# codename0og/codename-rvc-fork-3

Measured on AMD Instinct MI355X. Metric: 48 kHz audio samples/sec end-to-end VC, higher is better.
Workload: dtype f32 (vocoder ResBlock convs and upsamplers, HuBERT, RMVPE's U-Net convs: fp32 operands as exact bf16x3 splits on the bf16 matrix cores -- six products of order <= 2^-16 per multiply-add, fp32 accumulate; everything else fp32 / fp64)

## Files before the change

### codename-rvc-fork-3_amd/csrc/common.h

```cpp
#pragma once

#include <hip/hip_runtime.h>
#include <stdint.h>
#include <stdio.h>
#include <stdlib.h>
#include <string.h>

#include <string>

#include "bf16x3.h"
#include "rvc_amd.h"

namespace rvc {

void set_error(const char *fmt, ...);
int fail(const char *fmt, ...);

#define RVC_HIP(expr)                                                                         \
    do {                                                                                      \
        hipError_t _e = (expr);                                                               \
        if (_e != hipSuccess) return ::rvc::fail("%s failed: %s (%s:%d)", #expr, hipGetErrorString(_e), \
                                                 __FILE__, __LINE__);                         \
    } while (0)

// ... 20 lines not shown

static inline int64_t ceil_div(int64_t a, int64_t b) { return (a + b - 1) / b; }
static inline size_t align_up(size_t v, size_t a) { return (v + a - 1) / a * a; }

int cu_count();

struct PersistentGrid {
    int per_xcd;
    unsigned blocks;
};
static inline PersistentGrid persistent_grid(int64_t n_tiles) {
    const int per_xcd = (int)ceil_div(n_tiles, 8), cus_per_xcd = cu_count() / 8;
    return {per_xcd, 8u * (unsigned)(cus_per_xcd < per_xcd ? cus_per_xcd : per_xcd)};
}

static inline bool fits_2gib(int64_t elems, int elem_bytes) { return elems * elem_bytes < ((int64_t)1 << 31); }

int upload_packed(const char *fn, const void *host, size_t bytes, void *dev, void *stream);

typedef float f32x16 __attribute__((ext_vector_type(16)));
typedef float f32x4 __attribute__((ext_vector_type(4)));

__device__ __forceinline__ f32x16 mfma32(float a, float b, f32x16 c) {
    return __builtin_amdgcn_mfma_f32_32x32x2f32(a, b, c, 0, 0, 0);
}
__device__ __forceinline__ int mfma32_row(int reg, int lane) { return (reg & 3) + 8 * (reg >> 2) + 4 * (lane >> 5); }

__device__ __forceinline__ void lds_barrier() { asm volatile("s_waitcnt lgkmcnt(0)\n\ts_barrier" ::: "memory"); }

__device__ __forceinline__ float lrelu(float v, float slope) { return v > 0.f ? v : v * slope; }
// ... 3 lines not shown
```

### codename-rvc-fork-3_amd/csrc/convbf1.hip

```cpp
#include <stdlib.h>

#include <algorithm>
#include <mutex>
#include <type_traits>
#include <vector>

#include "conv.h"
#include "f16x2.h"

namespace rvc {

constexpr int CB1_NTH = 512;
constexpr int CB1_CK = 64;
constexpr int CB1_N1 = 64;

struct Cb1Bf16Taps {
    static constexpr const char *NAME = "convbf1";
    using frag = bf16x8;
    static constexpr bool PAIRS = false;
    static constexpr int PLANES = 3;
    static constexpr int TAPF = 1;
    static constexpr int NACC = 1;
    static constexpr int OUT_OPS = 24, VM_MAX = 56;
    static constexpr int tap_plane(int) { return 0; }
// ... 11 lines not shown
    static constexpr int tap_plane(int i) { return i == 2; }
    static constexpr int win_plane(int i) { return i == 0; }
    static constexpr int acc_of(int i) { return i != 1; }
};

struct Cb1Params {
    const float *x = nullptr;
    const void *u = nullptr;
    const float *bias = nullptr;
    const float *res = nullptr;
    const float *accin = nullptr;
    float *y = nullptr;
    int64_t L = 0;
    int dil = 1;
    float slope = 1.f, out_scale = 1.f;
    int tiles_per_row = 0, n_tiles = 0, per_xcd = 0;
};

template <int KW, int C, class F>
struct Cb1Geom {
    static constexpr int NCH = C / CB1_CK;
    static constexpr int RBW = C / 128;
    static constexpr int KS = CB1_CK / 16;
    static constexpr int NGC = KW * KS;
    static constexpr int NGT = NCH * NGC;
    static constexpr int H = (KW - 1) / 2;
    static constexpr int ROWB = 2 * F::PLANES * CB1_CK + 16;
    static constexpr int XROWS = CB1_N1 + (KW - 1) * 5;
    static constexpr int X_BYTES = (XROWS + 1) * ROWB;
    static constexpr int RC32 = (XROWS + 31) / 32;
    static constexpr int NIT = (CB1_CK / 8) * RC32 / 4;
    static constexpr int IO_BYTES = C * CB1_N1 * 4;
    static constexpr int LDS_BYTES = 2 * X_BYTES + IO_BYTES;
    static constexpr int ROWBLOCKS = C / 32;
    static constexpr int CONV_BYTES = NGT * ROWBLOCKS * F::TAPF * 1024;
    static constexpr int PA = F::TAPF == 1 ? 8 : 8 / RBW;
    static_assert(C == 128 || C == 256, "square layers of 128 or 256 channels");
    static_assert((CB1_CK / 8) * RC32 % 4 == 0, "the items must divide over the four stager waves");
    static_assert(4 * NIT + F::OUT_OPS <= F::VM_MAX, "memory operations in flight per stager wave");
    static_assert(LDS_BYTES <= 163840, "LDS budget");
    static_assert((ROWB / 16) % 2 == 1, "row stride must be an odd multiple of 16 bytes");
};

template <int KW, int C, class F>
__global__ void __launch_bounds__(CB1_NTH) __attribute__((amdgpu_waves_per_eu(2, 2)))
convbf1_kernel(const Cb1Params p) {
    using GM = Cb1Geom<KW, C, F>;
    using frag = typename F::frag;
    constexpr int NCH = GM::NCH, RBW = GM::RBW, KS = GM::KS, NGC = GM::NGC, NGT = GM::NGT, H = GM::H, ROWB = GM::ROWB, NIT = GM::NIT;
    constexpr int N1 = CB1_N1, CK = CB1_CK, PA = GM::PA, PLANES = F::PLANES, TAPF = F::TAPF, NACC = F::NACC;

    extern __shared__ __attribute__((aligned(16))) unsigned char cb_smem[];
    unsigned char *const xs = cb_smem;
    float *const io_lds = reinterpret_cast<float *>(cb_smem + 2 * GM::X_BYTES);

    const int tid = threadIdx.x, lane = tid & 63;
    const int wave = __builtin_amdgcn_readfirstlane(tid >> 6);
    const int half = lane >> 5, l31 = lane & 31;
    const int d = p.dil, XR = N1 + (KW - 1) * d;
    const int64_t L = p.L;
    const unsigned L4 = (unsigned)(L * 4);
    const int num_bytes = (int)((int64_t)C * L * 4);

    const int xcd = blockIdx.x & 7, slot = blockIdx.x >> 3, nslot = gridDim.x >> 3;
    const int tile_end = (xcd + 1) * p.per_xcd < p.n_tiles ? (xcd + 1) * p.per_xcd : p.n_tiles;
    const int tile0 = xcd * p.per_xcd + slot;
    if (tile0 >= tile_end) return;
    const int my_tiles = (tile_end - tile0 + nslot - 1) / nslot;
    const int n_q = my_tiles * NCH;

    if (wave >= 4) {
        __builtin_amdgcn_s_setprio(1);
        const int sw = wave - 4;
        float xr[NIT][4];
        constexpr int RC = GM::RC32;
        const int lq = lane >> 5;
        auto x_issue = [&](int q) __attribute__((always_inline)) {
            const int tl = tile0 + (q / NCH) * nslot, ch0 = (q % NCH) * CK;
            const int bb = tl / p.tiles_per_row;
            const int xt0 = (tl - bb * p.tiles_per_row) * N1 - H * d;
            const __amdgpu_buffer_rsrc_t rs = __builtin_amdgcn_make_buffer_rsrc((void *)(p.x + (int64_t)bb * C * L), 0, num_bytes, RSRC_RAW32);
            const unsigned Lu = (unsigned)L;
            int sw_o = sw;
            asm volatile("" : "+s"(sw_o));
#pragma unroll
            for (int i = 0; i < NIT; ++i) {
                const int wi = sw_o * NIT + i, qp = wi / RC, rc = wi - qp * RC;
                const int qd = 2 * qp + lq, r = rc * 32 + l31;
                const unsigned tg = (unsigned)(xt0 + r);
                const bool ok = r < XR && tg < Lu;
                const unsigned base = (unsigned)(ch0 + 4 * qd) * L4 + tg * 4u;
#pragma unroll
                for (int e = 0; e < 4; ++e)
// ... 78 lines not shown
                    }
                    if (l4) {
                        __builtin_amdgcn_raw_buffer_store_b128(__builtin_bit_cast(u32x4, f32x4{re[0], re[1], re[2], re[3]}), yrs, (int)o, 0, 0);
                    } else {
#pragma unroll
                        for (int e = 0; e < 4; ++e) {
                            const unsigned oe = (ok && t0 + 4 * chunk + e < L) ? o + 4u * (unsigned)e : BUF_OOB;
                            __builtin_amdgcn_raw_buffer_store_b32(__builtin_bit_cast(unsigned, re[e]), yrs, (int)oe, 0, 0);
                        }
                    }
                }
            }
        };
        x_issue(0);
        x_write(0);
        if (1 < n_q) x_issue(1);
        for (int q = 0; q < n_q; ++q) {
            lds_barrier();
            if (q % NCH == 0 && q > 0) out_store(tile0 + (q / NCH - 1) * nslot);
            if (q + 1 < n_q) x_write(q + 1);
            asm volatile("s_waitcnt vmcnt(8)" ::: "memory");
            if (q + 2 < n_q) x_issue(q + 2);
        }
        lds_barrier();
        out_store(tile0 + (my_tiles - 1) * nslot);
        return;
    }

    float bias[RBW][16];
    if constexpr (!F::PAIRS) {
#pragma unroll
        for (int rb = 0; rb < RBW; ++rb)
#pragma unroll
            for (int r = 0; r < 16; ++r) {
                const int ch = 32 * (RBW * wave + rb) + (r & 3) + 8 * (r >> 2) + 4 * half;
                bias[rb][r] = p.bias ? p.bias[ch] : 0.f;
            }
    }
    const __amdgpu_buffer_rsrc_t urs = __builtin_amdgcn_make_buffer_rsrc((void *)p.u, 0, GM::CONV_BYTES, RSRC_RAW32);
    frag fa[PA][RBW][TAPF];
// ... 9 lines not shown
        const int soff = (g * GM::ROWBLOCKS + RBW * wave) * TAPF * 1024;
        fa[slot_a][f / TAPF][f % TAPF] = __builtin_bit_cast(frag, __builtin_amdgcn_raw_buffer_load_b128(urs, 16 * lane + f * 1024, soff, 0));
    };
    auto load_b1 = [&](int buf, const unsigned char *src, int gc, int cb, int s) __attribute__((always_inline)) {
        const int tap = gc / KS, ks = gc - tap * KS;
        fb[buf][cb][s] = __builtin_bit_cast(frag, *reinterpret_cast<const u32x4 *>(src + tap * d * ROWB + ks * 32 + cb * 32 * ROWB + s * 2 * CK));
    };
#pragma unroll
    for (int g = 0; g < PA - 1; ++g) load_a(g, g);
    const int x_lane = l31 * ROWB + half * 16;
    float *const io_mine = io_lds + (32 * RBW * wave + 4 * half) * N1 + l31;
    constexpr int NM = 6 * RBW;

    static_assert((2 * NGC) % PA == 0 && NCH % 2 == 0, "two chunks of groups must be whole turns of the tap ring");
    int q = 0;
    for (int t = 0; t < my_tiles; ++t) {
#pragma unroll
        for (int rb = 0; rb < RBW; ++rb)
#pragma unroll
            for (int cb = 0; cb < 2; ++cb)
#pragma unroll
                for (int a = 0; a < NACC; ++a)
#pragma unroll
                    for (int r = 0; r < 16; ++r) acc[rb][cb][a][r] = 0.f;
#pragma unroll 1
        for (int cp = 0; cp < NCH / 2; ++cp) {
            const int g0 = cp * 2 * NGC;
#pragma unroll
            for (int c2 = 0; c2 < 2; ++c2, ++q) {
                lds_barrier();
                const unsigned char *const src = xs + (q & 1) * GM::X_BYTES + x_lane;
// ... 79 lines not shown
                            const int co = 32 * rb + (lane & 31), ci = CB1_CK * ch + 16 * ks + 8 * (lane >> 5) + e;
                            const size_t group = ((size_t)ch * k + tap) * KS + ks, at = (group * RB + rb) * planes * 512 + lane * 8 + e;
                            const float v = w[((size_t)co * c + ci) * k + tap];
                            if (fmt == CB1_F16X2) f16x2_split_host(v, &(*out)[at], &(*out)[at + 512]);
                            else (*out)[at] = bf16_rne(v);
                        }
    return 0;
}

template <int KW, int C, class F>
static int cb1_launch(Cb1Params p, int batch, hipStream_t stream) {
    if (reserve_whole_cu((const void *)convbf1_kernel<KW, C, F>, F::NAME)) return 1;
    p.tiles_per_row = (int)ceil_div(p.L, CB1_N1);
    p.n_tiles = p.tiles_per_row * batch;
    const PersistentGrid g = persistent_grid(p.n_tiles);
    p.per_xcd = g.per_xcd;
    hipLaunchKernelGGL((convbf1_kernel<KW, C, F>), dim3(g.blocks), dim3(CB1_NTH), LDS_WHOLE_CU, stream, p);
    RVC_LAUNCH_CHECK();
    return 0;
}

template <class F>
static int cb1_dispatch(const Cb1Params &p, int batch, int c, int k, hipStream_t stream) {
#define RVC_CB1_CASE(KW, CC) if (k == KW && c == CC) return cb1_launch<KW, CC, F>(p, batch, stream)
    RVC_CB1_CASE(3, 128); RVC_CB1_CASE(7, 128); RVC_CB1_CASE(11, 128);
    RVC_CB1_CASE(3, 256); RVC_CB1_CASE(7, 256); RVC_CB1_CASE(11, 256);
#undef RVC_CB1_CASE
    return fail("%s: unsupported shape c=%d k=%d", F::NAME, c, k);
}

int launch_convbf1(Cb1Format fmt, const float *x, const void *u, const float *bias, const float *res, const float *accin, float *y, int batch,
// ... 68 lines not shown
```

### codename-rvc-fork-3_amd/csrc/error.cpp

```cpp
#include <stdarg.h>

#include <map>
#include <mutex>
#include <unordered_map>

#include "common.h"

namespace rvc {

static thread_local char g_err[1024] = "";

void set_error(const char *fmt, ...) {
    va_list ap;
    va_start(ap, fmt);
    vsnprintf(g_err, sizeof(g_err), fmt, ap);
    va_end(ap);
}

int fail(const char *fmt, ...) {
    va_list ap;
    va_start(ap, fmt);
    vsnprintf(g_err, sizeof(g_err), fmt, ap);
    va_end(ap);
    return 1;
}

namespace {
struct DeviceState {
    int cus = 0;
    std::unordered_map<const void *, int> lds;
};
std::mutex g_dev_mu;
std::map<int, DeviceState> g_dev;
}

int reserve_lds(const void *kernel, int bytes, const char *what) {
    int dev = 0;
    RVC_HIP(hipGetDevice(&dev));
    std::lock_guard<std::mutex> g(g_dev_mu);
    int &granted = g_dev[dev].lds[kernel];
    if (bytes <= granted) return 0;
    const hipError_t e = hipFuncSetAttribute(kernel, hipFuncAttributeMaxDynamicSharedMemorySize, bytes);
    if (e != hipSuccess) return fail("%s: cannot reserve %d bytes of LDS on device %d: %s", what, bytes, dev, hipGetErrorString(e));
    granted = bytes;
    return 0;
}

int cu_count() {
    int dev = 0, cus = 0;
    if (hipGetDevice(&dev) != hipSuccess) return 256;
    std::lock_guard<std::mutex> g(g_dev_mu);
    DeviceState &d = g_dev[dev];
    if (!d.cus) d.cus = hipDeviceGetAttribute(&cus, hipDeviceAttributeMultiprocessorCount, dev) == hipSuccess && cus > 0 ? cus : 256;
    return d.cus;
}

int upload_packed(const char *fn, const void *host, size_t bytes, void *dev, void *stream) {
    hipError_t e = hipMemcpyAsync(dev, host, bytes, hipMemcpyHostToDevice, (hipStream_t)stream);
    if (e == hipSuccess) e = hipStreamSynchronize((hipStream_t)stream);
    if (e != hipSuccess) return fail("%s: %s", fn, hipGetErrorString(e));
    return 0;
}

}

extern "C" int rvc_abi_version(void) { return RVC_AMD_ABI_VERSION; }
extern "C" const char *rvc_last_error(void) { return rvc::g_err; }
```

### codename-rvc-fork-3_amd/csrc/resblock_bf.hip

```cpp
#include <stdlib.h>

#include <algorithm>
#include <atomic>
#include <mutex>
#include <type_traits>
#include <vector>

#include "conv.h"

namespace rvc {

constexpr int RBF_NTH = 512;

struct RbfParams {
    const float *x = nullptr;
    const void *u = nullptr;
    const float *b1 = nullptr, *b2 = nullptr;
    const float *accin = nullptr;
    float *y = nullptr;
    int64_t L = 0;
    int dil = 1;
    float slope = 1.f, out_scale = 1.f;
    int tiles_per_row = 0, n_tiles = 0, per_xcd = 0;
};

template <int KW, int C, int NTS = 3>
struct RbfGeom {
    static constexpr int KS = C / 16, RB = C / 32, CG = 4 / RB;
    static constexpr int N1 = CG * 64;
    static constexpr int H2 = (KW - 1) / 2;
    static constexpr int BN = (N1 - (KW - 1)) / 4 * 4;
    static constexpr int ROWB = 6 * C + 16;
    static constexpr int XROWS = N1 + (KW - 1) * 5;
    static constexpr int TROWS = N1 + (KW - 1);
    static constexpr int X_BYTES = (XROWS + 1) * ROWB, T_BYTES = TROWS * ROWB;
    static constexpr int RC32 = (XROWS + 31) / 32;
    static constexpr int NIT = (C / 8) * RC32 / 4;
    static constexpr int NG = KW * KS;
    static constexpr int GROUP_BYTES = NTS * 1024;
    static_assert(NTS == 1 || NTS == 3, "tap split: one term (bf16-valued taps) or three (fp32 taps)");
    static constexpr int CONV_BYTES = NG * RB * GROUP_BYTES;
    static constexpr int R_BYTES = C * N1 * 4 + 16;
    static constexpr int LDS_BYTES = X_BYTES + T_BYTES + R_BYTES;
    static_assert((C / 8) * RC32 % 4 == 0, "the items must divide over the four stager waves");
    static_assert(4 * NIT + 8 <= 56, "memory operations in flight per stager wave (kept below the 6-bit counter's range: see the stager's prologue)");
    static_assert(LDS_BYTES <= 163840, "LDS budget");
    static_assert((ROWB / 16) % 2 == 1, "row stride must be an odd multiple of 16 bytes");
};

template <int KW, int C, int DBG = 0, int NTS = 3>
__global__ void __launch_bounds__(RBF_NTH) __attribute__((amdgpu_waves_per_eu(2, 2)))
resblock_bf_kernel(const RbfParams p) {
    using GM = RbfGeom<KW, C, NTS>;
    constexpr int KS = GM::KS, RB = GM::RB, N1 = GM::N1, H2 = GM::H2, BN = GM::BN, ROWB = GM::ROWB, NIT = GM::NIT;
    constexpr int NG = GM::NG, PA = NTS == 1 ? 8 : 4;

    extern __shared__ __attribute__((aligned(16))) unsigned char rb_smem[];
    unsigned char *const xs = rb_smem;
    unsigned char *const ts = rb_smem + GM::X_BYTES;
    float *const io_lds = reinterpret_cast<float *>(rb_smem + GM::X_BYTES + GM::T_BYTES);

    const int tid = threadIdx.x, lane = tid & 63;
    const int wave = __builtin_amdgcn_readfirstlane(tid >> 6);
    const int half = lane >> 5, l31 = lane & 31;
    const int d = p.dil, h1 = H2 * d, XR = N1 + 2 * h1;
    const int64_t L = p.L;
    const unsigned L4 = (unsigned)(L * 4);
    const int num_bytes = (int)((int64_t)C * L * 4);

    const int xcd = blockIdx.x & 7, slot = blockIdx.x >> 3, nslot = gridDim.x >> 3;
    const int tile_end = (xcd + 1) * p.per_xcd < p.n_tiles ? (xcd + 1) * p.per_xcd : p.n_tiles;
    int tile = xcd * p.per_xcd + slot;
    if (tile >= tile_end) return;
    unsigned long long *const stamps = (DBG & 128) ? reinterpret_cast<unsigned long long *>(const_cast<float *>(p.accin)) + ((size_t)blockIdx.x * 2 + (wave >= 4 ? 1 : 0)) * 64 : nullptr;
    int n_stamp = 0;
    auto stamp = [&]() __attribute__((always_inline)) {
        if constexpr (DBG & 128) {
            if ((wave == 0 || wave == 4) && lane == 0 && n_stamp < 64) stamps[n_stamp] = __builtin_readcyclecounter();
            ++n_stamp;
        }
    };

    if (wave >= 4) {
        __builtin_amdgcn_s_setprio(1);
        const int ht = tid - 256, sw = wave - 4;
        constexpr int NSET = C == 32 ? 2 : 1;
        float xr[NSET][NIT][4];
        constexpr int RC = GM::RC32;
        const int lq = lane >> 5;
        auto x_issue = [&](auto SET, int tl) __attribute__((always_inline)) {
            constexpr int st = decltype(SET)::value;
            const int bb = tl / p.tiles_per_row;
            const int xt0 = (tl - bb * p.tiles_per_row) * BN - H2 - h1;
            const __amdgpu_buffer_rsrc_t rs = __builtin_amdgcn_make_buffer_rsrc((void *)(p.x + (int64_t)bb * C * L), 0, num_bytes, RSRC_RAW32);
            const unsigned Lu = (unsigned)L;
            int sw_o = sw;
            asm volatile("" : "+s"(sw_o));
#pragma unroll
            for (int i = 0; i < NIT; ++i) {
                const int wi = sw_o * NIT + i, qp = wi / RC, rc = wi - qp * RC;
                const int q = 2 * qp + lq, r = rc * 32 + l31;
// ... 78 lines not shown
                        re[e] = mul_np(re[e], out_scale);
                    }
                    if (l4) {
                        __builtin_amdgcn_raw_buffer_store_b128(__builtin_bit_cast(u32x4, f32x4{re[0], re[1], re[2], re[3]}), yrs, (int)o, 0, 0);
                    } else {
#pragma unroll
                        for (int e = 0; e < 4; ++e) {
                            const unsigned oe = (ok && t0 + 4 * chunk + e < L) ? o + 4u * (unsigned)e : BUF_OOB;
                            __builtin_amdgcn_raw_buffer_store_b32(__builtin_bit_cast(unsigned, re[e]), yrs, (int)oe, 0, 0);
                        }
                    }
                }
            }
        };
        const bool has_acc = p.accin != nullptr && !(DBG & 128);
        for (int o = ht * 16; o < (KW - 1) * ROWB; o += 256 * 16) *reinterpret_cast<u32x4 *>(ts + N1 * ROWB + o) = u32x4{0u, 0u, 0u, 0u};
        constexpr std::integral_constant<int, 0> S0{};
        constexpr std::integral_constant<int, NSET - 1> SL{};
        x_issue(S0, tile);
        x_write(S0);
        if (NSET == 2 && tile + nslot < tile_end) x_issue(SL, tile + nslot);
        int prev = -1;
        auto phase = [&](int tl, auto SET_CUR, auto SET_NEXT) __attribute__((always_inline)) {
            stamp();
            lds_barrier();
            stamp();
            lds_barrier();
            if (prev >= 0) out_store(prev, has_acc);
            asm volatile("s_waitcnt vmcnt(8)" ::: "memory");
            if (tl + NSET * nslot < tile_end) x_issue(SET_CUR, tl + NSET * nslot);
            stamp();
            lds_barrier();
            stamp();
            if constexpr (DBG & 128) asm volatile("s_waitcnt vmcnt(0)" ::: "memory");
            stamp();
            if (tl + nslot < tile_end) x_write(SET_NEXT);
            stamp();
            n_stamp += 2;
            prev = tl;
        };
        for (; tile < tile_end; tile += 2 * nslot) {
            phase(tile, S0, SL);
            if (tile + nslot < tile_end) phase(tile + nslot, SL, S0);
        }
        lds_barrier();
        asm volatile("s_waitcnt vmcnt(0)" ::: "memory");
        lds_barrier();
        out_store(prev, has_acc);
        return;
    }

    const int rb = wave % RB, cg = wave / RB;
    const int col0 = cg * 64;
    float bias1[16], bias2[16];
#pragma unroll
    for (int r = 0; r < 16; ++r) {
        const int ch = 32 * rb + (r & 3) + 8 * (r >> 2) + 4 * half;
        bias1[r] = p.b1 ? p.b1[ch] : 0.f;
        bias2[r] = p.b2 ? p.b2[ch] : 0.f;
    }
    const __amdgpu_buffer_rsrc_t urs = __builtin_amdgcn_make_buffer_rsrc((void *)p.u, 0, 2 * GM::CONV_BYTES, RSRC_RAW32);
    const float slope = p.slope;

// ... 58 lines not shown
#pragma unroll
        for (int cb = 0; cb < 2; ++cb)
#pragma unroll
            for (int r = 0; r < 16; ++r) rsd[cb][r] = io_mine[((r & 3) + 8 * (r >> 2)) * N1 + cb * 32];
#pragma unroll
        for (int cb = 0; cb < 2; ++cb)
#pragma unroll
            for (int r = 0; r < 16; ++r) io_mine[((r & 3) + 8 * (r >> 2)) * N1 + cb * 32] = io[cb][r];
#pragma unroll
        for (int cb = 0; cb < 2; ++cb)
#pragma unroll
            for (int r = 0; r < 16; ++r) io[cb][r] = rsd[cb][r];
    };

    a_prologue(0);
    for (; tile < tile_end; tile += nslot) {
        const int bb = tile / p.tiles_per_row;
        const int64_t t0 = (int64_t)(tile - bb * p.tiles_per_row) * BN;
        stamp();
        lds_barrier();
        stamp();
        swap_io();
        stamp();
        lds_barrier();
        stamp();
        conv_loop(0, xsrc, xstep);
        stamp();
        a_prologue(1);
#pragma unroll
        for (int cb = 0; cb < 2; ++cb) {
            const int j = col0 + cb * 32 + l31;
// ... 75 lines not shown
                            const size_t group = (((size_t)cv * k + tap) * KS + ks) * RB + rb;
                            uint16_t h[3];
                            bf16_split_host(w[((size_t)co * c + ci) * k + tap], tap_splits, h);
                            for (int s = 0; s < tap_splits; ++s) (*out)[(group * tap_splits + s) * 512 + lane * 8 + e] = h[s];
                        }
    }
}

template <int KW, int C, int DBG = 0, int NTS = 3>
static int rbf_launch(RbfParams p, int batch, hipStream_t stream) {
    using GM = RbfGeom<KW, C, NTS>;
    if (reserve_whole_cu((const void *)resblock_bf_kernel<KW, C, DBG, NTS>, "resblock_bf")) return 1;
    p.tiles_per_row = (int)ceil_div(p.L, GM::BN);
    p.n_tiles = p.tiles_per_row * batch;
    const PersistentGrid g = persistent_grid(p.n_tiles);
    p.per_xcd = g.per_xcd;
    hipLaunchKernelGGL((resblock_bf_kernel<KW, C, DBG, NTS>), dim3(g.blocks), dim3(RBF_NTH), LDS_WHOLE_CU, stream, p);
    RVC_LAUNCH_CHECK();
    return 0;
}

int launch_resblock_bf(const float *x, const void *u, const float *b1, const float *b2, const float *accin, float *y, int batch, int c,
                       int64_t L, int k, int dil, float slope, float out_scale, hipStream_t stream, int tap_splits) {
    if (!resblock_bf_supported(c, k, dil)) return fail("resblock_bf: unsupported shape (%d channels, %d taps, dilation %d)", c, k, dil);
    if (tap_splits != 1 && tap_splits != 3) return fail("resblock_bf: tap split of %d terms (1 or 3)", tap_splits);
    if (x == y) return fail("resblock_bf: in-place operation is not supported");
    if (!(slope >= 0.f && slope <= 1.f)) return fail("resblock_bf: leaky slope %g outside [0, 1]", (double)slope);
    if (!resblock_bf_fits(c, L)) return fail("resblock_bf: a %d x %lld slab exceeds the 2 GiB buffer addressing", c, (long long)L);
    if (L <= 0 || batch <= 0) return 0;
    if ((int64_t)ceil_div(L, 64) * batch >= ((int64_t)1 << 30)) return fail("resblock_bf: too many tiles");
    RbfParams p;
// ... 71 lines not shown
```

### codename-rvc-fork-3_amd/csrc/upsbf.hip

```cpp
#include <stdlib.h>

#include <algorithm>
#include <mutex>
#include <type_traits>
#include <vector>

#include "conv.h"

namespace rvc {

constexpr int UB_NTH = 512;
constexpr int UB_CK = 64;

struct UbParams {
    const float *x = nullptr;
    const float *har = nullptr;
    const void *u = nullptr;
    const float *bias = nullptr;
    float *y = nullptr;
    int64_t L_in = 0, L_out = 0, Lh = 0;
    int c_in = 0, c_out = 0;
    int n_xchunks = 0;
    int vk = 0;
    int S = 0, P = 0;
    int pad = 0;
    float slope = 0.1f;
    int n_mblk = 0, col_tiles = 0, n_tiles = 0, per_xcd = 0;
};

template <int R, int MB>
struct UbGeom {
    static constexpr int RB_T = MB / 32;
    static constexpr int RBW = RB_T >= 4 ? RB_T / 4 : 1;
    static constexpr int CG = RB_T >= 4 ? 1 : 4 / RB_T;
    static constexpr int N1 = 64 * CG;
    static constexpr int W = N1 * R;
    static constexpr int CPB = (MB - 1) / R + 2;
    static constexpr int KS = UB_CK / 16;
    static constexpr int NGC = 2 * KS;
    static constexpr int PA = 4;
    static constexpr int ROWB = 6 * UB_CK + 16;
    static constexpr int XROWS = N1 + 1;
    static constexpr int X_BYTES = (XROWS + 1) * ROWB;
    static constexpr int RC32 = (XROWS + 31) / 32;
    static constexpr int NIT = (UB_CK / 8) * RC32 / 4;
    static constexpr int IO_FLOATS = CPB * W;
    static constexpr int IO_BYTES = IO_FLOATS * 4 + 16;
    static constexpr int LDS_BYTES = 2 * X_BYTES + IO_BYTES;
    static constexpr int GROUP_BYTES = RB_T * 3 * 1024;
    static_assert(MB == 64 || MB == 128 || MB == 256, "GEMM rows per tile");
    static_assert(R >= 1 && R <= MB, "a channel's phases span at most two m-blocks");
    static_assert((UB_CK / 8) * RC32 % 4 == 0, "the items must divide over the four stager waves");
    static_assert(NGC % PA == 0 && KS % PA == 0, "a chunk's groups must be whole turns of the tap ring");
    static_assert(LDS_BYTES <= 163840, "LDS budget");
};

template <int R, int MB>
__global__ void __launch_bounds__(UB_NTH) __attribute__((amdgpu_waves_per_eu(2, 2)))
upsbf_kernel(const UbParams p) {
    using GM = UbGeom<R, MB>;
    constexpr int RB_T = GM::RB_T, RBW = GM::RBW, N1 = GM::N1, W = GM::W, KS = GM::KS, NGC = GM::NGC, PA = GM::PA, ROWB = GM::ROWB;
    constexpr int NIT = GM::NIT, CK = UB_CK;

    extern __shared__ __attribute__((aligned(16))) unsigned char ub_smem[];
    unsigned char *const xs = ub_smem;
    float *const io_lds = reinterpret_cast<float *>(ub_smem + 2 * GM::X_BYTES);

    const int tid = threadIdx.x, lane = tid & 63;
    const int wave = __builtin_amdgcn_readfirstlane(tid >> 6);
    const int half = lane >> 5, l31 = lane & 31;
    const int64_t L_in = p.L_in, L_out = p.L_out;
    const int nxc = p.n_xchunks, ncht = nxc + (p.vk > 0 ? 1 : 0);
    const int ngt = nxc * NGC + (p.vk > 0 ? KS : 0);
    const int n_mblk = p.n_mblk;
    const int m_total = p.c_out * R;

    const int xcd = blockIdx.x & 7, slot = blockIdx.x >> 3, nslot = gridDim.x >> 3;
    const int tile_end = (xcd + 1) * p.per_xcd < p.n_tiles ? (xcd + 1) * p.per_xcd : p.n_tiles;
    const int tile0 = xcd * p.per_xcd + slot;
    if (tile0 >= tile_end) return;
    const int my_tiles = (tile_end - tile0 + nslot - 1) / nslot;
    const int n_q = my_tiles * ncht;
    auto tile_coords = [&](int tl, int &mblk, int &ct, int &bb) __attribute__((always_inline)) {
        mblk = tl % n_mblk;
        const int rest = tl / n_mblk;
        bb = rest / p.col_tiles;
        ct = rest - bb * p.col_tiles;
    };

    for (int o = tid * 16; o < 2 * GM::X_BYTES; o += UB_NTH * 16) *reinterpret_cast<u32x4 *>(xs + o) = u32x4{0u, 0u, 0u, 0u};
    lds_barrier();
    const int nqp_noise = (p.vk + 1 + 7) / 8;

    if (wave >= 4) {
        __builtin_amdgcn_s_setprio(1);
        const int sw = wave - 4, ht = tid - 256;
        float xr[NIT][4];
        constexpr int RC = GM::RC32;
        const int lq = lane >> 5;
        const unsigned L4 = (unsigned)(L_in * 4);
        const int x_bytes = (int)((int64_t)p.c_in * L_in * 4);
        auto x_issue = [&](int tl, int ci) __attribute__((always_inline)) {
            int mblk, ct, bb;
            tile_coords(tl, mblk, ct, bb);
            const int q0m1 = ct * N1 - 1;
            int sw_o = sw;
// ... 77 lines not shown
                    const int64_t t = t_base + i;
                    const int m = (co0 + row) * R + i % R;
                    const bool ok = f < n_el && m >= m0 && m < m0 + MB && m < m_total && t >= 0 && t < L_out;
                    v[k] = io_lds[f < n_el ? f : 0];
                    bv[k] = !fold && p.bias && ok ? p.bias[co0 + row] : 0.f;
                    off[k] = ok ? (unsigned)(co0 + row) * Lo4 + (unsigned)t * 4u : BUF_OOB;
                }
#pragma unroll
                for (int k = 0; k < 4; ++k) __builtin_amdgcn_raw_buffer_store_b32(__builtin_bit_cast(unsigned, v[k] + bv[k]), yrs, (int)off[k], 0, 0);
            }
        };
        int wt = 0, wc = 0, it = 0, ic = 0;
        auto adv = [&](int &t_, int &c_) __attribute__((always_inline)) {
            if (++c_ == ncht) { c_ = 0; ++t_; }
        };
        x_issue(tile0, 0);
        x_write(0, 0);
        adv(wt, wc); adv(it, ic);
        if (1 < n_q) x_issue(tile0 + it * nslot, ic);
        adv(it, ic);
        int ct_i = 0, cc_i = 0;
        for (int q = 0; q < n_q; ++q) {
            lds_barrier();
            if (cc_i == 0 && q > 0) out_store(tile0 + (ct_i - 1) * nslot);
            if (ncht == 1) lds_barrier();
            if (q + 1 < n_q) x_write(q + 1, wc);
            adv(wt, wc);
            asm volatile("s_waitcnt vmcnt(8)" ::: "memory");
            if (q + 2 < n_q) x_issue(tile0 + it * nslot, ic);
            adv(it, ic);
            adv(ct_i, cc_i);
        }
        lds_barrier();
        out_store(tile0 + (my_tiles - 1) * nslot);
        return;
    }

    const int rb0 = RB_T >= 4 ? RBW * wave : wave % RB_T;
    const int col0 = RB_T >= 4 ? 0 : 64 * (wave / RB_T);
    const __amdgpu_buffer_rsrc_t urs = __builtin_amdgcn_make_buffer_rsrc((void *)p.u, 0, n_mblk * ngt * GM::GROUP_BYTES, RSRC_RAW32);
    bf16x8 fa[PA][RBW][3];
    bf16x8 fb[2][2][3];
    f32x16 acc[RBW][2];
    auto load_a1 = [&](int slot_a, int byte_off, int rb, int s) __attribute__((always_inline)) {
        fa[slot_a][rb][s] = __builtin_bit_cast(bf16x8, __builtin_amdgcn_raw_buffer_load_b128(urs, 16 * lane + ((rb0 + rb) * 3 + s) * 1024, byte_off, 0));
    };
    auto load_b1 = [&](int buf, const unsigned char *src, int gc, int cb, int s) __attribute__((always_inline)) {
        const int j = gc / KS, ks = gc - j * KS;
        fb[buf][cb][s] = __builtin_bit_cast(bf16x8, *reinterpret_cast<const u32x4 *>(src + (1 - j) * ROWB + ks * 32 + cb * 32 * ROWB + s * 2 * CK));
    };
    const int x_lane = (col0 + l31) * ROWB + half * 16;
    constexpr int ia6[6] = {0, 1, 0, 2, 1, 0}, ib6[6] = {2, 1, 1, 0, 0, 0};
    constexpr int NM = 12 * RBW;

    int mblk, ct, bb;
    tile_coords(tile0, mblk, ct, bb);
    int a_base = mblk * ngt * GM::GROUP_BYTES;
#pragma unroll
    for (int g = 0; g < PA - 1; ++g)
#pragma unroll
        for (int rb = 0; rb < RBW; ++rb)
#pragma unroll
            for (int s = 0; s < 3; ++s) load_a1(g, a_base + g * GM::GROUP_BYTES, rb, s);

    int q = 0;
    for (int t = 0; t < my_tiles; ++t) {
        const int tl = tile0 + t * nslot;
        tile_coords(tl, mblk, ct, bb);
        a_base = mblk * ngt * GM::GROUP_BYTES;
        int a_next = a_base;
        if (t + 1 < my_tiles) {
            int m2, c2, b2;
            tile_coords(tl + nslot, m2, c2, b2);
            a_next = m2 * ngt * GM::GROUP_BYTES;
        }
#pragma unroll
        for (int rb = 0; rb < RBW; ++rb)
#pragma unroll
            for (int cb = 0; cb < 2; ++cb)
#pragma unroll
                for (int r = 0; r < 16; ++r) acc[rb][cb][r] = 0.f;
        int g0 = 0;
#pragma unroll 1
        for (int c = 0; c < ncht; ++c, ++q) {
            const bool noise = c == nxc;
            lds_barrier();
            const unsigned char *const src = xs + (q & 1) * GM::X_BYTES + x_lane;
#pragma unroll
// ... 99 lines not shown
                            const int k = kq - ph * nc_stride;
                            float v = row_ok && kq < vk && k >= 0 && k < nc_k ? nw[(size_t)co * nc_k + k] : 0.f;
                            if (row_ok && kq == vk && bias) v = bias[co];
                            put((size_t)mblk * ngt + nxc * 8 + ks, rb, lane, e, v);
                        }
            }
}

template <int R, int MB>
static int ub_launch(UbParams p, int batch, hipStream_t stream) {
    using GM = UbGeom<R, MB>;
    if (reserve_whole_cu((const void *)upsbf_kernel<R, MB>, "upsbf")) return 1;
    p.col_tiles = (int)ceil_div(p.L_in + 1, GM::N1);
    p.n_tiles = p.col_tiles * p.n_mblk * batch;
    const PersistentGrid g = persistent_grid(p.n_tiles);
    p.per_xcd = g.per_xcd;
    hipLaunchKernelGGL((upsbf_kernel<R, MB>), dim3(g.blocks), dim3(UB_NTH), LDS_WHOLE_CU, stream, p);
    RVC_LAUNCH_CHECK();
    return 0;
}

int launch_upsbf(const float *x, const float *har, int64_t Lh, const void *u, const float *bias, float *y, int batch, int c_in, int c_out,
                 int64_t L_in, int64_t L_out, int rate, int ksize, int pad, int vk, int64_t S, int64_t P, float slope, hipStream_t stream) {
    if (!upsbf_supported(c_in, c_out, rate, ksize, vk)) return fail("upsbf: unsupported shape (%d -> %d channels, rate %d, kernel %d, %d noise rows)", c_in, c_out, rate, ksize, vk);
    if (vk > 0 && (!har || Lh <= 0 || !fits_2gib(Lh, 4) || S > 4096 || P > 65536)) return fail("upsbf: bad noise source");
    if (!fits_2gib((int64_t)c_in * L_in, 4) || !fits_2gib((int64_t)c_out * L_out, 4)) return fail("upsbf: slab exceeds the 2 GiB buffer addressing");
    if (L_in <= 0 || batch <= 0) return 0;
    UbParams p;
    p.x = x; p.har = har; p.u = u; p.bias = bias; p.y = y; p.L_in = L_in; p.L_out = L_out; p.Lh = vk > 0 ? Lh : 0;
    p.c_in = c_in; p.c_out = c_out; p.n_xchunks = c_in / UB_CK; p.vk = vk; p.S = (int)S; p.P = (int)P; p.pad = pad; p.slope = slope;
    int mb, ngt;
// ... 50 lines not shown
```

Measured before the change: 61.46 million.

## Replace static persistent tile striding with atomic per-XCD tile claiming and work stealing

Persistent conv, resblock and upsampler kernels now take tiles dynamically from per-XCD atomic counters instead of a fixed stride. Each block prefers its home XCD's range and steals from other XCDs once that range runs dry. Tile indices go into a small LDS ring so the stager and MFMA waves can prefetch ahead, and the last block to finish resets the counters. The aim is to cut tail imbalance between blocks, at the cost of atomic traffic, extra readfirstlane LDS reads and a per-stream counter pool.

```diff
diff --git a/codename-rvc-fork-3_amd/csrc/common.h b/codename-rvc-fork-3_amd/csrc/common.h
--- a/codename-rvc-fork-3_amd/csrc/common.h
+++ b/codename-rvc-fork-3_amd/csrc/common.h
@@ -58,6 +58,107 @@
     return {per_xcd, 8u * (unsigned)(cus_per_xcd < per_xcd ? cus_per_xcd : per_xcd)};
 }
 
+constexpr int CLAIM_WORDS = 16, CLAIM_DONE = 8;
+struct TileClaim {
+    unsigned *ctr = nullptr;
+    int n_tiles = 0, per_xcd = 0;
+};
+int tile_claim_counters(hipStream_t stream, unsigned **ctr);
+static inline int tile_claim(hipStream_t stream, int64_t n_tiles, const PersistentGrid &g, TileClaim *c) {
+    c->n_tiles = (int)n_tiles;
+    c->per_xcd = g.per_xcd;
+    c->ctr = nullptr;
+    if (!knob("RVC_TILE_CLAIM", 1)) return 0;
+    return tile_claim_counters(stream, &c->ctr);
+}
+
+#ifdef __HIPCC__
+struct TileClaimer {
+    int home = 0, tried = 0;
+    unsigned left = 0xffu;
+    int next = 0, step = 0, end = 0;
+};
+__device__ __forceinline__ TileClaimer tile_claimer(const TileClaim &c) {
+    TileClaimer s;
+    s.home = blockIdx.x & 7;
+    const int hi = (s.home + 1) * c.per_xcd;
+    s.next = s.home * c.per_xcd + (int)(blockIdx.x >> 3);
+    s.step = (int)(gridDim.x >> 3);
+    s.end = hi < c.n_tiles ? hi : c.n_tiles;
+    return s;
+}
+__device__ __forceinline__ void claim_range(const TileClaim &c, const TileClaimer &s, int &x, int &lo, int &len) {
+    x = (s.home + s.tried) & 7;
+    lo = x * c.per_xcd;
+    const int hi = lo + c.per_xcd < c.n_tiles ? lo + c.per_xcd : c.n_tiles;
+    len = hi > lo ? hi - lo : 0;
+}
+__device__ __forceinline__ unsigned claim_issue(const TileClaim &c, TileClaimer &s) {
+#ifdef RVC_ABLATE
+    if (!c.ctr) return 0u;
+#endif
+    while (s.tried < 8) {
+        int x, lo, len;
+        claim_range(c, s, x, lo, len);
+        if (len > 0 && (s.left >> x & 1u)) return atomicAdd(c.ctr + x, 1u);
+        ++s.tried;
+    }
+    return 0u;
+}
+__device__ __forceinline__ int claim_take(const TileClaim &c, TileClaimer &s, unsigned drawn) {
+#ifdef RVC_ABLATE
+    if (!c.ctr) {
+        const int t = s.next;
+        s.next += s.step;
+        return t < s.end ? t : -1;
+    }
+#endif
+    while (s.tried < 8) {
+        int x, lo, len;
+        claim_range(c, s, x, lo, len);
+        if (drawn < (unsigned)len) return lo + (int)drawn;
+        if (s.tried++ == 0) {
+            unsigned seen[8];
+#pragma unroll
+            for (int r = 0; r < 8; ++r) seen[r] = __hip_atomic_load(c.ctr + r, __ATOMIC_RELAXED, __HIP_MEMORY_SCOPE_AGENT);
+            s.left = 0u;
+#pragma unroll
+            for (int r = 0; r < 8; ++r) {
+                const int hi = (r + 1) * c.per_xcd < c.n_tiles ? (r + 1) * c.per_xcd : c.n_tiles;
+                if ((int)seen[r] < hi - r * c.per_xcd) s.left |= 1u << r;
+            }
+        }
+        drawn = claim_issue(c, s);
+    }
+    return -1;
+}
+__device__ __forceinline__ int claim_tile(const TileClaim &c, TileClaimer &s) { return claim_take(c, s, claim_issue(c, s)); }
+template <int N>
+__device__ __forceinline__ void claim_first(const TileClaim &c, TileClaimer &s, int *q) {
+    const int lane = threadIdx.x & 63;
+    int t = -1;
+    if (lane < N) {
+#ifdef RVC_ABLATE
+        if (!c.ctr) s.next += lane * s.step;
+#endif
+        t = claim_tile(c, s);
+    }
+#ifdef RVC_ABLATE
+    if (!c.ctr) s.next = s.home * c.per_xcd + (int)(blockIdx.x >> 3) + N * s.step;
+#endif
+    const unsigned long long got = __ballot(t >= 0);
+    const int below = __popcll(got & ((1ull << lane) - 1ull));
+    if (lane < N) q[t >= 0 ? below : __popcll(got) + lane - below] = t;
+}
+__device__ __forceinline__ void claim_done(const TileClaim &c) {
+#ifdef RVC_ABLATE
+    if (!c.ctr) return;
+#endif
+    if (atomicAdd(c.ctr + CLAIM_DONE, 1u) == gridDim.x - 1)
+        for (int i = 0; i <= CLAIM_DONE; ++i) atomicExch(c.ctr + i, 0u);
+}
+#endif
+
 static inline bool fits_2gib(int64_t elems, int elem_bytes) { return elems * elem_bytes < ((int64_t)1 << 31); }
 
 int upload_packed(const char *fn, const void *host, size_t bytes, void *dev, void *stream);
diff --git a/codename-rvc-fork-3_amd/csrc/convbf1.hip b/codename-rvc-fork-3_amd/csrc/convbf1.hip
--- a/codename-rvc-fork-3_amd/csrc/convbf1.hip
+++ b/codename-rvc-fork-3_amd/csrc/convbf1.hip
@@ -49,7 +49,8 @@
     int64_t L = 0;
     int dil = 1;
     float slope = 1.f, out_scale = 1.f;
-    int tiles_per_row = 0, n_tiles = 0, per_xcd = 0;
+    int tiles_per_row = 0, n_tiles = 0;
+    TileClaim claim;
 };
 
 template <int KW, int C, class F>
@@ -73,7 +74,7 @@
     static_assert(C == 128 || C == 256, "square layers of 128 or 256 channels");
     static_assert((CB1_CK / 8) * RC32 % 4 == 0, "the items must divide over the four stager waves");
     static_assert(4 * NIT + F::OUT_OPS <= F::VM_MAX, "memory operations in flight per stager wave");
-    static_assert(LDS_BYTES <= 163840, "LDS budget");
+    static_assert(LDS_BYTES + 16 <= 163840, "LDS budget (+ the queue of tile indices)");
     static_assert((ROWB / 16) % 2 == 1, "row stride must be an odd multiple of 16 bytes");
 };
 
@@ -97,12 +98,15 @@
     const unsigned L4 = (unsigned)(L * 4);
     const int num_bytes = (int)((int64_t)C * L * 4);
 
-    const int xcd = blockIdx.x & 7, slot = blockIdx.x >> 3, nslot = gridDim.x >> 3;
-    const int tile_end = (xcd + 1) * p.per_xcd < p.n_tiles ? (xcd + 1) * p.per_xcd : p.n_tiles;
-    const int tile0 = xcd * p.per_xcd + slot;
-    if (tile0 >= tile_end) return;
-    const int my_tiles = (tile_end - tile0 + nslot - 1) / nslot;
-    const int n_q = my_tiles * NCH;
+    int *const tq = reinterpret_cast<int *>(cb_smem + GM::LDS_BYTES);
+    auto tq_at = [&](int t) __attribute__((always_inline)) { return __builtin_amdgcn_readfirstlane(tq[t & 3]); };
+    TileClaimer cl = tile_claimer(p.claim);
+    if (wave == 4) claim_first<2>(p.claim, cl, tq);
+    lds_barrier();
+    if (tq_at(0) < 0) {
+        if (wave == 4 && lane == 0) claim_done(p.claim);
+        return;
+    }
 
     if (wave >= 4) {
         __builtin_amdgcn_s_setprio(1);
@@ -111,7 +115,7 @@
         constexpr int RC = GM::RC32;
         const int lq = lane >> 5;
         auto x_issue = [&](int q) __attribute__((always_inline)) {
-            const int tl = tile0 + (q / NCH) * nslot, ch0 = (q % NCH) * CK;
+            const int tl = tq_at(q / NCH), ch0 = (q % NCH) * CK;
             const int bb = tl / p.tiles_per_row;
             const int xt0 = (tl - bb * p.tiles_per_row) * N1 - H * d;
             const __amdgpu_buffer_rsrc_t rs = __builtin_amdgcn_make_buffer_rsrc((void *)(p.x + (int64_t)bb * C * L), 0, num_bytes, RSRC_RAW32);
@@ -220,16 +224,33 @@
         };
         x_issue(0);
         x_write(0);
-        if (1 < n_q) x_issue(1);
-        for (int q = 0; q < n_q; ++q) {
+        x_issue(1);
+        int cur = tq_at(0), prev = -1;
+        unsigned drawn = 0u;
+        bool pending = false, more = false;
+        for (int q = 0; cur >= 0; ++q) {
             lds_barrier();
-            if (q % NCH == 0 && q > 0) out_store(tile0 + (q / NCH - 1) * nslot);
-            if (q + 1 < n_q) x_write(q + 1);
+            if (q % NCH == 0 && q > 0) out_store(prev);
+            if (tq_at((q + 1) / NCH) >= 0) x_write(q + 1);
+            if (pending) {
+                if (wave == 4 && lane == 0) tq[(q / NCH + 2) & 3] = more ? claim_take(p.claim, cl, drawn) : -1;
+                pending = false;
+            }
             asm volatile("s_waitcnt vmcnt(8)" ::: "memory");
-            if (q + 2 < n_q) x_issue(q + 2);
+            if (q % NCH == 0) {
+                more = tq_at(q / NCH + 1) >= 0;
+                if (wave == 4 && lane == 0 && more) drawn = claim_issue(p.claim, cl);
+                pending = true;
+            }
+            if (tq_at((q + 2) / NCH) >= 0) x_issue(q + 2);
+            if ((q + 1) % NCH == 0) {
+                prev = cur;
+                cur = tq_at((q + 1) / NCH);
+            }
         }
         lds_barrier();
-        out_store(tile0 + (my_tiles - 1) * nslot);
+        out_store(prev);
+        if (wave == 4 && lane == 0) claim_done(p.claim);
         return;
     }
 
@@ -269,7 +290,7 @@
 
     static_assert((2 * NGC) % PA == 0 && NCH % 2 == 0, "two chunks of groups must be whole turns of the tap ring");
     int q = 0;
-    for (int t = 0; t < my_tiles; ++t) {
+    for (int t = 0; tq_at(t) >= 0; ++t) {
 #pragma unroll
         for (int rb = 0; rb < RBW; ++rb)
 #pragma unroll
@@ -379,7 +400,7 @@
     p.tiles_per_row = (int)ceil_div(p.L, CB1_N1);
     p.n_tiles = p.tiles_per_row * batch;
     const PersistentGrid g = persistent_grid(p.n_tiles);
-    p.per_xcd = g.per_xcd;
+    if (tile_claim(stream, p.n_tiles, g, &p.claim)) return 1;
     hipLaunchKernelGGL((convbf1_kernel<KW, C, F>), dim3(g.blocks), dim3(CB1_NTH), LDS_WHOLE_CU, stream, p);
     RVC_LAUNCH_CHECK();
     return 0;
diff --git a/codename-rvc-fork-3_amd/csrc/error.cpp b/codename-rvc-fork-3_amd/csrc/error.cpp
--- a/codename-rvc-fork-3_amd/csrc/error.cpp
+++ b/codename-rvc-fork-3_amd/csrc/error.cpp
@@ -29,7 +29,12 @@
 struct DeviceState {
     int cus = 0;
     std::unordered_map<const void *, int> lds;
+    std::unordered_map<hipStream_t, unsigned *> claim;
+    unsigned *claim_pool = nullptr;
+    int claim_used = 0;
 };
+constexpr int CLAIM_SLOT_WORDS = 64;
+constexpr int CLAIM_SLOTS = 256;
 std::mutex g_dev_mu;
 std::map<int, DeviceState> g_dev;
 }
@@ -55,6 +60,44 @@
     return d.cus;
 }
 
+static int claim_pool_new(unsigned **pool) {
+    hipStreamCaptureMode mode = hipStreamCaptureModeRelaxed;
+    RVC_HIP(hipThreadExchangeStreamCaptureMode(&mode));
+    const size_t bytes = (size_t)CLAIM_SLOTS * CLAIM_SLOT_WORDS * sizeof(unsigned);
+    hipStream_t s = nullptr;
+    hipError_t e = hipMalloc((void **)pool, bytes);
+    if (e == hipSuccess) e = hipStreamCreateWithFlags(&s, hipStreamNonBlocking);
+    if (e == hipSuccess) e = hipMemsetAsync(*pool, 0, bytes, s);
+    if (e == hipSuccess) e = hipStreamSynchronize(s);
+    if (s) (void)hipStreamDestroy(s);
+    (void)hipThreadExchangeStreamCaptureMode(&mode);
+    if (e != hipSuccess) return fail("tile-claim counters: %s", hipGetErrorString(e));
+    return 0;
+}
+
+int tile_claim_counters(hipStream_t stream, unsigned **ctr) {
+    static_assert(CLAIM_WORDS <= CLAIM_SLOT_WORDS, "a slot holds one stream's counters");
+    int dev = 0;
+    RVC_HIP(hipGetDevice(&dev));
+    std::lock_guard<std::mutex> g(g_dev_mu);
+    DeviceState &d = g_dev[dev];
+    unsigned *&mine = d.claim[stream];
+    if (!mine) {
+        if (!d.claim_pool || d.claim_used == CLAIM_SLOTS) {
+            unsigned *pool = nullptr;
+            if (claim_pool_new(&pool)) {
+                d.claim.erase(stream);
+                return 1;
+            }
+            d.claim_pool = pool;
+            d.claim_used = 0;
+        }
+        mine = d.claim_pool + (size_t)d.claim_used++ * CLAIM_SLOT_WORDS;
+    }
+    *ctr = mine;
+    return 0;
+}
+
 int upload_packed(const char *fn, const void *host, size_t bytes, void *dev, void *stream) {
     hipError_t e = hipMemcpyAsync(dev, host, bytes, hipMemcpyHostToDevice, (hipStream_t)stream);
     if (e == hipSuccess) e = hipStreamSynchronize((hipStream_t)stream);
diff --git a/codename-rvc-fork-3_amd/csrc/resblock_bf.hip b/codename-rvc-fork-3_amd/csrc/resblock_bf.hip
--- a/codename-rvc-fork-3_amd/csrc/resblock_bf.hip
+++ b/codename-rvc-fork-3_amd/csrc/resblock_bf.hip
@@ -21,7 +21,8 @@
     int64_t L = 0;
     int dil = 1;
     float slope = 1.f, out_scale = 1.f;
-    int tiles_per_row = 0, n_tiles = 0, per_xcd = 0;
+    int tiles_per_row = 0, n_tiles = 0;
+    TileClaim claim;
 };
 
 template <int KW, int C, int NTS = 3>
@@ -44,7 +45,7 @@
     static constexpr int LDS_BYTES = X_BYTES + T_BYTES + R_BYTES;
     static_assert((C / 8) * RC32 % 4 == 0, "the items must divide over the four stager waves");
     static_assert(4 * NIT + 8 <= 56, "memory operations in flight per stager wave (kept below the 6-bit counter's range: see the stager's prologue)");
-    static_assert(LDS_BYTES <= 163840, "LDS budget");
+    static_assert(LDS_BYTES + 16 <= 163840, "LDS budget (+ the queue of tile indices)");
     static_assert((ROWB / 16) % 2 == 1, "row stride must be an odd multiple of 16 bytes");
 };
 
@@ -68,10 +69,9 @@
     const unsigned L4 = (unsigned)(L * 4);
     const int num_bytes = (int)((int64_t)C * L * 4);
 
-    const int xcd = blockIdx.x & 7, slot = blockIdx.x >> 3, nslot = gridDim.x >> 3;
-    const int tile_end = (xcd + 1) * p.per_xcd < p.n_tiles ? (xcd + 1) * p.per_xcd : p.n_tiles;
-    int tile = xcd * p.per_xcd + slot;
-    if (tile >= tile_end) return;
+    constexpr int NSET = C == 32 ? 2 : 1;
+    int *const tq = reinterpret_cast<int *>(rb_smem + GM::LDS_BYTES);
+    auto tq_at = [&](int i) __attribute__((always_inline)) { return __builtin_amdgcn_readfirstlane(tq[i & 3]); };
     unsigned long long *const stamps = (DBG & 128) ? reinterpret_cast<unsigned long long *>(const_cast<float *>(p.accin)) + ((size_t)blockIdx.x * 2 + (wave >= 4 ? 1 : 0)) * 64 : nullptr;
     int n_stamp = 0;
     auto stamp = [&]() __attribute__((always_inline)) {
@@ -84,7 +84,6 @@
     if (wave >= 4) {
         __builtin_amdgcn_s_setprio(1);
         const int ht = tid - 256, sw = wave - 4;
-        constexpr int NSET = C == 32 ? 2 : 1;
         float xr[NSET][NIT][4];
         constexpr int RC = GM::RC32;
         const int lq = lane >> 5;
@@ -193,39 +192,55 @@
             }
         };
         const bool has_acc = p.accin != nullptr && !(DBG & 128);
+        TileClaimer cl = tile_claimer(p.claim);
+        if (wave == 4) claim_first<NSET + 1>(p.claim, cl, tq);
         for (int o = ht * 16; o < (KW - 1) * ROWB; o += 256 * 16) *reinterpret_cast<u32x4 *>(ts + N1 * ROWB + o) = u32x4{0u, 0u, 0u, 0u};
+        lds_barrier();
+        const int tile = tq_at(0);
+        if (tile < 0) {
+            if (wave == 4 && lane == 0) claim_done(p.claim);
+            return;
+        }
         constexpr std::integral_constant<int, 0> S0{};
         constexpr std::integral_constant<int, NSET - 1> SL{};
         x_issue(S0, tile);
         x_write(S0);
-        if (NSET == 2 && tile + nslot < tile_end) x_issue(SL, tile + nslot);
+        if (NSET == 2 && tq_at(1) >= 0) x_issue(SL, tq_at(1));
         int prev = -1;
-        auto phase = [&](int tl, auto SET_CUR, auto SET_NEXT) __attribute__((always_inline)) {
+        auto phase = [&](int i, auto SET_CUR, auto SET_NEXT) __attribute__((always_inline)) {
+            const int tl = tq_at(i);
             stamp();
             lds_barrier();
             stamp();
             lds_barrier();
             if (prev >= 0) out_store(prev, has_acc);
             asm volatile("s_waitcnt vmcnt(8)" ::: "memory");
-            if (tl + NSET * nslot < tile_end) x_issue(SET_CUR, tl + NSET * nslot);
+            const int ahead = tq_at(i + NSET);
+            if (ahead >= 0) x_issue(SET_CUR, ahead);
+            unsigned drawn = 0u;
+            if (wave == 4 && lane == 0 && ahead >= 0) drawn = claim_issue(p.claim, cl);
             stamp();
             lds_barrier();
             stamp();
             if constexpr (DBG & 128) asm volatile("s_waitcnt vmcnt(0)" ::: "memory");
             stamp();
-            if (tl + nslot < tile_end) x_write(SET_NEXT);
+            if (tq_at(i + 1) >= 0) x_write(SET_NEXT);
+            if (wave == 4 && lane == 0) tq[(i + NSET + 1) & 3] = ahead >= 0 ? claim_take(p.claim, cl, drawn) : -1;
             stamp();
             n_stamp += 2;
             prev = tl;
         };
-        for (; tile < tile_end; tile += 2 * nslot) {
-            phase(tile, S0, SL);
-            if (tile + nslot < tile_end) phase(tile + nslot, SL, S0);
+        for (int i = 0;; i += 2) {
+            phase(i, S0, SL);
+            if (tq_at(i + 1) < 0) break;
+            phase(i + 1, SL, S0);
+            if (tq_at(i + 2) < 0) break;
         }
         lds_barrier();
         asm volatile("s_waitcnt vmcnt(0)" ::: "memory");
         lds_barrier();
         out_store(prev, has_acc);
+        if (wave == 4 && lane == 0) claim_done(p.claim);
         return;
     }
 
@@ -314,7 +329,11 @@
     };
 
     a_prologue(0);
-    for (; tile < tile_end; tile += nslot) {
+    lds_barrier();
+    if (tq_at(0) < 0) return;
+    for (int i = 0;; ++i) {
+        const int tile = tq_at(i);
+        if (tile < 0) break;
         const int bb = tile / p.tiles_per_row;
         const int64_t t0 = (int64_t)(tile - bb * p.tiles_per_row) * BN;
         stamp();
@@ -420,7 +439,7 @@
     p.tiles_per_row = (int)ceil_div(p.L, GM::BN);
     p.n_tiles = p.tiles_per_row * batch;
     const PersistentGrid g = persistent_grid(p.n_tiles);
-    p.per_xcd = g.per_xcd;
+    if (tile_claim(stream, p.n_tiles, g, &p.claim)) return 1;
     hipLaunchKernelGGL((resblock_bf_kernel<KW, C, DBG, NTS>), dim3(g.blocks), dim3(RBF_NTH), LDS_WHOLE_CU, stream, p);
     RVC_LAUNCH_CHECK();
     return 0;
diff --git a/codename-rvc-fork-3_amd/csrc/upsbf.hip b/codename-rvc-fork-3_amd/csrc/upsbf.hip
--- a/codename-rvc-fork-3_amd/csrc/upsbf.hip
+++ b/codename-rvc-fork-3_amd/csrc/upsbf.hip
@@ -25,7 +25,8 @@
     int S = 0, P = 0;
     int pad = 0;
     float slope = 0.1f;
-    int n_mblk = 0, col_tiles = 0, n_tiles = 0, per_xcd = 0;
+    int n_mblk = 0, col_tiles = 0, n_tiles = 0;
+    TileClaim claim;
 };
 
 template <int R, int MB>
@@ -52,7 +53,7 @@
     static_assert(R >= 1 && R <= MB, "a channel's phases span at most two m-blocks");
     static_assert((UB_CK / 8) * RC32 % 4 == 0, "the items must divide over the four stager waves");
     static_assert(NGC % PA == 0 && KS % PA == 0, "a chunk's groups must be whole turns of the tap ring");
-    static_assert(LDS_BYTES <= 163840, "LDS budget");
+    static_assert(LDS_BYTES + 16 <= 163840, "LDS budget (+ the queue of tile indices)");
 };
 
 template <int R, int MB>
@@ -75,12 +76,10 @@
     const int n_mblk = p.n_mblk;
     const int m_total = p.c_out * R;
 
-    const int xcd = blockIdx.x & 7, slot = blockIdx.x >> 3, nslot = gridDim.x >> 3;
-    const int tile_end = (xcd + 1) * p.per_xcd < p.n_tiles ? (xcd + 1) * p.per_xcd : p.n_tiles;
-    const int tile0 = xcd * p.per_xcd + slot;
-    if (tile0 >= tile_end) return;
-    const int my_tiles = (tile_end - tile0 + nslot - 1) / nslot;
-    const int n_q = my_tiles * ncht;
+    int *const tq = reinterpret_cast<int *>(ub_smem + GM::LDS_BYTES);
+    auto tq_at = [&](int t) __attribute__((always_inline)) { return __builtin_amdgcn_readfirstlane(tq[t & 3]); };
+    TileClaimer cl = tile_claimer(p.claim);
+    if (wave == 4) claim_first<3>(p.claim, cl, tq);
     auto tile_coords = [&](int tl, int &mblk, int &ct, int &bb) __attribute__((always_inline)) {
         mblk = tl % n_mblk;
         const int rest = tl / n_mblk;
@@ -90,6 +89,10 @@
 
     for (int o = tid * 16; o < 2 * GM::X_BYTES; o += UB_NTH * 16) *reinterpret_cast<u32x4 *>(xs + o) = u32x4{0u, 0u, 0u, 0u};
     lds_barrier();
+    if (tq_at(0) < 0) {
+        if (wave == 4 && lane == 0) claim_done(p.claim);
+        return;
+    }
     const int nqp_noise = (p.vk + 1 + 7) / 8;
 
     if (wave >= 4) {
@@ -197,25 +200,44 @@
         auto adv = [&](int &t_, int &c_) __attribute__((always_inline)) {
             if (++c_ == ncht) { c_ = 0; ++t_; }
         };
-        x_issue(tile0, 0);
+        x_issue(tq_at(0), 0);
         x_write(0, 0);
         adv(wt, wc); adv(it, ic);
-        if (1 < n_q) x_issue(tile0 + it * nslot, ic);
+        if (tq_at(it) >= 0) x_issue(tq_at(it), ic);
         adv(it, ic);
         int ct_i = 0, cc_i = 0;
-        for (int q = 0; q < n_q; ++q) {
+        int cur = tq_at(0), prev = -1;
+        unsigned drawn = 0u;
+        bool pending = false, more = false;
+        auto take = [&]() __attribute__((always_inline)) {
+            if (wave == 4 && lane == 0) tq[(ct_i + 3) & 3] = more ? claim_take(p.claim, cl, drawn) : -1;
+            pending = false;
+        };
+        for (int q = 0; cur >= 0; ++q) {
             lds_barrier();
-            if (cc_i == 0 && q > 0) out_store(tile0 + (ct_i - 1) * nslot);
+            if (cc_i == 0 && q > 0) out_store(prev);
             if (ncht == 1) lds_barrier();
-            if (q + 1 < n_q) x_write(q + 1, wc);
+            if (tq_at(wt) >= 0) x_write(q + 1, wc);
             adv(wt, wc);
+            if (pending) take();
             asm volatile("s_waitcnt vmcnt(8)" ::: "memory");
-            if (q + 2 < n_q) x_issue(tile0 + it * nslot, ic);
+            if (cc_i == 0) {
+                more = tq_at(ct_i + 2) >= 0;
+                if (wave == 4 && lane == 0 && more) drawn = claim_issue(p.claim, cl);
+                pending = true;
+            }
+            if (tq_at(it) >= 0) x_issue(tq_at(it), ic);
             adv(it, ic);
+            if (ncht == 1) take();
             adv(ct_i, cc_i);
+            if (cc_i == 0) {
+                prev = cur;
+                cur = tq_at(ct_i);
+            }
         }
         lds_barrier();
-        out_store(tile0 + (my_tiles - 1) * nslot);
+        out_store(prev);
+        if (wave == 4 && lane == 0) claim_done(p.claim);
         return;
     }
 
@@ -237,7 +259,7 @@
     constexpr int NM = 12 * RBW;
 
     int mblk, ct, bb;
-    tile_coords(tile0, mblk, ct, bb);
+    tile_coords(tq_at(0), mblk, ct, bb);
     int a_base = mblk * ngt * GM::GROUP_BYTES;
 #pragma unroll
     for (int g = 0; g < PA - 1; ++g)
@@ -247,14 +269,15 @@
             for (int s = 0; s < 3; ++s) load_a1(g, a_base + g * GM::GROUP_BYTES, rb, s);
 
     int q = 0;
-    for (int t = 0; t < my_tiles; ++t) {
-        const int tl = tile0 + t * nslot;
+    for (int t = 0;; ++t) {
+        const int tl = tq_at(t), tl_next = tq_at(t + 1);
+        if (tl < 0) break;
         tile_coords(tl, mblk, ct, bb);
         a_base = mblk * ngt * GM::GROUP_BYTES;
         int a_next = a_base;
-        if (t + 1 < my_tiles) {
+        if (tl_next >= 0) {
             int m2, c2, b2;
-            tile_coords(tl + nslot, m2, c2, b2);
+            tile_coords(tl_next, m2, c2, b2);
             a_next = m2 * ngt * GM::GROUP_BYTES;
         }
 #pragma unroll
@@ -384,7 +407,7 @@
     p.col_tiles = (int)ceil_div(p.L_in + 1, GM::N1);
     p.n_tiles = p.col_tiles * p.n_mblk * batch;
     const PersistentGrid g = persistent_grid(p.n_tiles);
-    p.per_xcd = g.per_xcd;
+    if (tile_claim(stream, p.n_tiles, g, &p.claim)) return 1;
     hipLaunchKernelGGL((upsbf_kernel<R, MB>), dim3(g.blocks), dim3(UB_NTH), LDS_WHOLE_CU, stream, p);
     RVC_LAUNCH_CHECK();
     return 0;
```

New measurement: 60.97 million. About the same (-0.8%).
